# zkemail/zk-email-verify

Measured on NVIDIA H100. Metric: EmailVerifier proofs/sec (witness+prove), higher is better.
Workload: dtype u256 (BN254 Fr/Fq integers, 8x32-bit limbs)

## Files before the change

### zk-email-verify_b200/csrc/engine.cu

```cuda
#include "ff.cuh"
namespace zke { namespace dev { unsigned long long g_kernel_launches = 0; } }
#include "witness.cu"
#include "matvec.cu"
#include "ntt.cu"
#include "msm.cuh"
#include "fixed_base.cuh"
namespace zke { namespace dev {
ZKE_DEFINE_CONSTANT_UPLOAD(upload_constants_engine)
cudaError_t upload_constants_msm_g1(const FieldConsts*, const FieldConsts*);
cudaError_t upload_constants_msm_g2(const FieldConsts*, const FieldConsts*);
cudaError_t upload_constants_fixed_base(const FieldConsts*, const FieldConsts*);
cudaError_t upload_constants_verify(const FieldConsts*, const FieldConsts*);
} }

#include "../../include/zkemail_b200.h"
#include "cuda_host.hpp"
#include "engine.hpp"
#include "witness_program.hpp"
#include "binfile.hpp"
#include "ec_host.hpp"
#include "setup_host.hpp"
#include <algorithm>
#include <cstdio>
#include <cstring>
// ... 766 lines not shown
static void sync_lanes(zke_ctx* x) {
    cudaStreamSynchronize(x->stream);
    for (int i = 0; i < x->lanes_alloc; ++i) { cudaStreamSynchronize(x->lanes[i].st); cudaStreamSynchronize(x->lanes[i].heavy); }
}

static void enqueue_prove(zke_ctx* x, zke_ctx::Slot& S, size_t batch, const uint8_t* rs) {
    const zke_zkey* zk = x->zkey;
    if (!zk) throw std::runtime_error("context was opened without a proving key");
    if (batch == 0 || batch > S.loaded) throw std::runtime_error("no witness loaded for this batch (call zke_witness first)");
    if (rs) {
        for (size_t e = 0; e < 2 * batch; ++e) {
            U256 v;
            memcpy(v.v, rs + 32 * e, 32);
            if (u256_cmp(v, fr_params().p) >= 0) throw std::runtime_error("r / s not reduced mod the group order");
        }
        S.rs.assign(rs, rs + 64 * batch);
    } else {
        S.rs.clear();
    }
    CUDA_OK(cudaSetDevice(x->device));
    const uint32_t N = 1u << zk->log_n, m = x->n_vars, l = x->n_public;
    const bool prof = x->profile;
    const int n_lanes = prof ? 1 : x->n_lanes;
    if (const char* e = getenv("ZKE_SPLIT_STREAMS")) x->split_streams = atoi(e) != 0;
    if (l) CUDA_OK(cudaMemcpy2DAsync(S.publics_host, (size_t)l * 32, S.w_all.p + 32, x->stride * 32, (size_t)l * 32, batch, cudaMemcpyDeviceToHost, x->stream));
    CUDA_OK(cudaEventRecord(S.witness_done, x->stream));
    for (int i = 0; i < n_lanes; ++i) CUDA_OK(cudaStreamWaitEvent(x->lanes[i].st, S.witness_done, 0));
    for (size_t e = 0; e < batch; ++e) {
        zke_ctx::Lane& L = x->lanes[e % n_lanes];
        cudaStream_t st = L.st;
        const uint8_t* w = S.w_all.p + 32 * x->stride * e;
        uint8_t* res = S.results.p + (size_t)ZKE_RESULT_STRIDE * e;
        uint32_t* flag = (uint32_t*)(res + ZKE_RES_FLAG_OFF);
        size_t t0 = 0, t1 = 0;
        CUDA_OK(cudaMemsetAsync(flag, 0xff, 4, st));
        if (prof) t0 = x->mark(st);
        cudaStream_t hv = (prof || !x->split_streams) ? st : L.heavy;
        dev::launch_build_ab(x->r1cs, w, L.va.p, L.vb.p, L.vc.p, N, flag, st);
        if (prof) { t1 = x->mark(st); x->spans.push_back({ZKE_STAGE_MATVEC, t0, t1}); t0 = t1; }
        if (hv != st) { CUDA_OK(cudaEventRecord(L.ev[0], st)); CUDA_OK(cudaStreamWaitEvent(hv, L.ev[0], 0)); }
        dev::launch_intt_dif(L.va.p, x->ntt, x->coset_scale.p, hv);
        dev::launch_intt_dif(L.vb.p, x->ntt, x->coset_scale.p, hv);
        dev::launch_intt_dif(L.vc.p, x->ntt, x->coset_scale.p, hv);
        dev::launch_ntt_dit(L.va.p, x->ntt, hv);
        dev::launch_ntt_dit(L.vb.p, x->ntt, hv);
        dev::launch_ntt_dit(L.vc.p, x->ntt, hv);
        dev::launch_quotient(L.va.p, L.vb.p, L.vc.p, L.vd.p, N, hv);
        CHECK_LAUNCH();
        if (hv != st) CUDA_OK(cudaEventRecord(L.ev[1], hv));
        if (prof) { t1 = x->mark(st); x->spans.push_back({ZKE_STAGE_NTT, t0, t1}); t0 = t1; }
        uint8_t* ws_w = L.msm_ws.p;
        dev::MsmPlan<dev::Fq>::run(zk->A.p, w, m, x->cfg_w, ws_w, res + 0 * ZKE_RES_G1_BLOCK, st);
        if (prof) { t1 = x->mark(st); x->spans.push_back({ZKE_STAGE_MSM_A, t0, t1}); t0 = t1; }
        dev::MsmPlan<dev::Fq>::run(zk->B1.p, w, m, x->cfg_w, ws_w, res + 1 * ZKE_RES_G1_BLOCK, st);
        if (prof) { t1 = x->mark(st); x->spans.push_back({ZKE_STAGE_MSM_B1, t0, t1}); t0 = t1; }
        dev::MsmPlan<dev::Fq>::run(zk->C.p, w, m, x->cfg_w, ws_w, res + 2 * ZKE_RES_G1_BLOCK, st);
        if (prof) { t1 = x->mark(st); x->spans.push_back({ZKE_STAGE_MSM_C, t0, t1}); t0 = t1; }
        dev::MsmPlan<dev::Fq2>::run(zk->B2.p, w, m, x->cfg_w, ws_w, res + 4 * ZKE_RES_G1_BLOCK, st);
        CHECK_LAUNCH();
        if (prof) { t1 = x->mark(st); x->spans.push_back({ZKE_STAGE_MSM_B2, t0, t1}); t0 = t1; }
        if (hv != st) CUDA_OK(cudaStreamWaitEvent(st, L.ev[1], 0));
        {
            dev::MsmPlan<dev::Fq>::Heavy heavy{hv, L.ev[2], L.ev[3]};
            if (prof) {
                size_t i0, i1;
                cudaEvent_t evs[2];
                evs[0] = x->ev(&i0); evs[1] = x->ev(&i1);
                dev::MsmPlan<dev::Fq>::run(zk->H.p, L.vd.p, N, x->cfg_h, L.msm_ws.p, res + 3 * ZKE_RES_G1_BLOCK, st, evs, &heavy);
                x->spans.push_back({ZKE_STAGE_MSM_H_BUCKETS, i0, i1});
                t1 = x->mark(st); x->spans.push_back({ZKE_STAGE_MSM_H, t0, t1}); t0 = t1;
            } else {
                dev::MsmPlan<dev::Fq>::run(zk->H.p, L.vd.p, N, x->cfg_h, L.msm_ws.p, res + 3 * ZKE_RES_G1_BLOCK, st, nullptr, &heavy);
            }
        }
        CHECK_LAUNCH();
        CUDA_OK(cudaMemcpyAsync(S.results_host + (size_t)ZKE_RESULT_STRIDE * e, res, ZKE_RESULT_STRIDE, cudaMemcpyDeviceToHost, st));
        CUDA_OK(cudaEventRecord(S.done[e], st));
    }
    S.batch = (uint32_t)batch;
}

static int finish_prove(zke_ctx* x, zke_ctx::Slot& S, uint8_t* proofs_out, uint8_t* publics_out, int32_t* status, std::string& msg) {
    const zke_zkey* zk = x->zkey;
    const size_t batch = S.batch;
    const uint32_t l = x->n_public;
    const G1JacH alpha1 = G1JacH::from_affine(zk->alpha1), beta1 = G1JacH::from_affine(zk->beta1), delta1 = G1JacH::from_affine(zk->delta1);
    const G2JacH beta2 = G2JacH::from_affine(zk->beta2), delta2 = G2JacH::from_affine(zk->delta2);
    std::vector<int32_t> st_local(batch, -1);
    std::string first_error;
    std::mutex err_mutex;
    auto one = [&](size_t e) {
        CUDA_OK(cudaEventSynchronize(S.done[e]));
        const uint8_t* res = S.results_host + (size_t)ZKE_RESULT_STRIDE * e;
        uint32_t flag;
        memcpy(&flag, res + ZKE_RES_FLAG_OFF, 4);
        const int32_t s = flag == 0xffffffffu ? -1 : (int32_t)flag;
        st_local[e] = s;
        uint8_t* out = proofs_out + 256 * e;
        if (s >= 0) { memset(out, 0, 256); return; }
        U256 r, sc;
        if (!S.rs.empty()) { memcpy(r.v, S.rs.data() + 64 * e, 32); memcpy(sc.v, S.rs.data() + 64 * e + 32, 32); }
        else { random_scalar(r); random_scalar(sc); }
        G1AffineH ma = finish_msm<Fq>(res + 0 * ZKE_RES_G1_BLOCK, x->cfg_w);
        G1AffineH mb1 = finish_msm<Fq>(res + 1 * ZKE_RES_G1_BLOCK, x->cfg_w);
        G1AffineH mc = finish_msm<Fq>(res + 2 * ZKE_RES_G1_BLOCK, x->cfg_w);
        G1AffineH mh = finish_msm<Fq>(res + 3 * ZKE_RES_G1_BLOCK, x->cfg_h);
        G2AffineH mb2 = finish_msm<Fq2>(res + 4 * ZKE_RES_G1_BLOCK, x->cfg_w);
        G1JacH pa = alpha1.add(G1JacH::from_affine(ma)).add(delta1.mul(r));
        G2JacH pb2 = beta2.add(G2JacH::from_affine(mb2)).add(delta2.mul(sc));
        G1JacH pb1 = beta1.add(G1JacH::from_affine(mb1)).add(delta1.mul(sc));
        U256 rs_prod = (Fr::from_u256(r) * Fr::from_u256(sc)).to_u256();
        G1JacH pc = G1JacH::from_affine(mc).add(G1JacH::from_affine(mh)).add(pa.mul(sc)).add(pb1.mul(r)).add(delta1.mul(rs_prod).neg());
        G1AffineH A = pa.to_affine(), C = pc.to_affine();
// ... 110 lines not shown
    map.log_cols = log_cols; map.log_m = log_m; map.col0 = col0;
    const uint32_t n_rows = (uint32_t)world << log_cols;
    dev::launch_build_ab(x->r1cs, S.w_all.p, L.va.p, L.vb.p, L.vc.p, n_rows, flag, st, &map);
    const uint32_t n_cols = 1u << log_cols;
    dev::launch_intt_cross(L.va.p, x->ntt, log_g, col0, n_cols, st);
    dev::launch_intt_cross(L.vb.p, x->ntt, log_g, col0, n_cols, st);
    dev::launch_intt_cross(L.vc.p, x->ntt, log_g, col0, n_cols, st);
    CHECK_LAUNCH();
    CUDA_OK(cudaStreamSynchronize(st));
    x->shard_stage = 1;
}

static void shard_mid(zke_ctx* x) {
    if (x->shard_stage != 1) throw std::runtime_error("zke_shard_mid out of order");
    CUDA_OK(cudaSetDevice(x->device));
    int log_m, log_cols; uint32_t col0;
    shard_geometry(x, log_m, log_cols, col0);
    zke_ctx::Lane& L = x->lanes[0];
    cudaStream_t st = L.st;
    const size_t block_off = ((size_t)x->shard_rank << log_m);
    for (uint8_t* v : {L.va.p, L.vb.p, L.vc.p}) {
        dev::launch_intt_dif_block(v + 32 * block_off, x->ntt, log_m, x->coset_scale.p + (x->ntt.shoup ? 64 : 32) * block_off, st);
        dev::launch_ntt_dit_block(v + 32 * block_off, x->ntt, log_m, st);
    }
    CHECK_LAUNCH();
    CUDA_OK(cudaStreamSynchronize(st));
    x->shard_stage = 2;
}

static void put_g1(uint8_t* dst, const G1AffineH& p) { write_fq(dst, p.x); write_fq(dst + 32, p.y); }

static void shard_end(zke_ctx* x, uint8_t* partial_out, uint8_t* publics_out) {
    if (x->shard_stage != 2) throw std::runtime_error("zke_shard_end out of order");
    const zke_zkey* zk = x->zkey;
    CUDA_OK(cudaSetDevice(x->device));
    int log_m, log_cols; uint32_t col0;
    shard_geometry(x, log_m, log_cols, col0);
    zke_ctx::Slot& S = x->slots[0];
    zke_ctx::Lane& L = x->lanes[0];
    cudaStream_t st = L.st;
    const uint32_t N = 1u << zk->log_n, m = x->n_vars, l = x->n_public;
    const int G = x->shard_world, log_g = x->shard_log_g;
    const uint32_t n_cols = 1u << log_cols;
    dev::launch_ntt_cross(L.va.p, x->ntt, log_g, col0, n_cols, st);
    dev::launch_ntt_cross(L.vb.p, x->ntt, log_g, col0, n_cols, st);
    dev::launch_ntt_cross(L.vc.p, x->ntt, log_g, col0, n_cols, st);
    CUDA_OK(cudaMemsetAsync(L.vd.p, 0, (size_t)N * 32, st));
    dev::launch_quotient_cols(L.va.p, L.vb.p, L.vc.p, L.vd.p, (int)zk->log_n, log_g, col0, (uint32_t)log_cols, st);
    CHECK_LAUNCH();
    const uint32_t lo = (uint32_t)((uint64_t)m * x->shard_rank / G), hi = (uint32_t)((uint64_t)m * (x->shard_rank + 1) / G);
    const uint8_t* w = S.w_all.p;
    uint8_t* res = S.results.p;
    dev::MsmPlan<dev::Fq>::run(zk->A.p + 64ull * lo, w + 32ull * lo, hi - lo, x->cfg_w, L.msm_ws.p, res + 0 * ZKE_RES_G1_BLOCK, st);
    dev::MsmPlan<dev::Fq>::run(zk->B1.p + 64ull * lo, w + 32ull * lo, hi - lo, x->cfg_w, L.msm_ws.p, res + 1 * ZKE_RES_G1_BLOCK, st);
    dev::MsmPlan<dev::Fq>::run(zk->C.p + 64ull * lo, w + 32ull * lo, hi - lo, x->cfg_w, L.msm_ws.p, res + 2 * ZKE_RES_G1_BLOCK, st);
    dev::MsmPlan<dev::Fq2>::run(zk->B2.p + 128ull * lo, w + 32ull * lo, hi - lo, x->cfg_w, L.msm_ws.p, res + 4 * ZKE_RES_G1_BLOCK, st);
    dev::MsmPlan<dev::Fq>::run(zk->H.p, L.vd.p, N, x->cfg_h, L.msm_ws.p, res + 3 * ZKE_RES_G1_BLOCK, st);
    CHECK_LAUNCH();
    CUDA_OK(cudaMemcpyAsync(S.results_host, res, ZKE_RESULT_STRIDE, cudaMemcpyDeviceToHost, st));
    if (l) CUDA_OK(cudaMemcpyAsync(S.publics_host, S.w_all.p + 32, (size_t)l * 32, cudaMemcpyDeviceToHost, st));
    CUDA_OK(cudaStreamSynchronize(st));
    const uint8_t* rh = S.results_host;
    put_g1(partial_out + 0, finish_msm<Fq>(rh + 0 * ZKE_RES_G1_BLOCK, x->cfg_w));
    put_g1(partial_out + 64, finish_msm<Fq>(rh + 1 * ZKE_RES_G1_BLOCK, x->cfg_w));
    put_g1(partial_out + 128, finish_msm<Fq>(rh + 2 * ZKE_RES_G1_BLOCK, x->cfg_w));
    put_g1(partial_out + 192, finish_msm<Fq>(rh + 3 * ZKE_RES_G1_BLOCK, x->cfg_h));
    const G2AffineH b2 = finish_msm<Fq2>(rh + 4 * ZKE_RES_G1_BLOCK, x->cfg_w);
    write_fq(partial_out + 256, b2.x.c0); write_fq(partial_out + 288, b2.x.c1); write_fq(partial_out + 320, b2.y.c0); write_fq(partial_out + 352, b2.y.c1);
    memcpy(partial_out + 384, rh + ZKE_RES_FLAG_OFF, 4);
    if (publics_out && l) memcpy(publics_out, S.publics_host, (size_t)l * 32);
    x->shard_stage = 0;
}

static Fq fq_from_le(const uint8_t* b) {
    U256 v;
    memcpy(v.v, b, 32);
    if (u256_cmp(v, fq_params().p) >= 0) throw std::runtime_error("partial point coordinate not reduced");
    return Fq::from_u256(v);
}

struct ShardKeyPoints { G1AffineH alpha1, beta1, delta1; G2AffineH beta2, delta2; };
static int shard_combine(const ShardKeyPoints* zk, const uint8_t* partials, int world, const uint8_t* rs, uint8_t* out, int32_t* status) {
    G1JacH sa = G1JacH::inf(), sb1 = G1JacH::inf(), sc = G1JacH::inf(), sh = G1JacH::inf();
    G2JacH sb2 = G2JacH::inf();
    uint32_t first_bad = 0xffffffffu;
    for (int r = 0; r < world; ++r) {
        const uint8_t* p = partials + (size_t)ZKE_SHARD_PARTIAL_BYTES * r;
        auto g1 = [&](const uint8_t* q) { return G1AffineH{fq_from_le(q), fq_from_le(q + 32)}; };
        const G1AffineH a = g1(p), b1 = g1(p + 64), c = g1(p + 128), h = g1(p + 192);
        const G2AffineH b2{Fq2{fq_from_le(p + 256), fq_from_le(p + 288)}, Fq2{fq_from_le(p + 320), fq_from_le(p + 352)}};
        if (!g1_on_curve(a) || !g1_on_curve(b1) || !g1_on_curve(c) || !g1_on_curve(h) || !g2_on_curve(b2)) throw std::runtime_error("partial point not on the curve");
        sa = sa.add_affine(a); sb1 = sb1.add_affine(b1); sc = sc.add_affine(c); sh = sh.add_affine(h); sb2 = sb2.add_affine(b2);
        uint32_t f;
        memcpy(&f, p + 384, 4);
        first_bad = std::min(first_bad, f);
    }
    if (status) *status = first_bad == 0xffffffffu ? -1 : (int32_t)first_bad;
    if (first_bad != 0xffffffffu) { memset(out, 0, 256); return 1; }
    U256 r, s;
    if (rs) { memcpy(r.v, rs, 32); memcpy(s.v, rs + 32, 32); }
    else { random_scalar(r); random_scalar(s); }
    if (u256_cmp(r, fr_params().p) >= 0 || u256_cmp(s, fr_params().p) >= 0) throw std::runtime_error("r / s not reduced mod the group order");
    const G1JacH alpha1 = G1JacH::from_affine(zk->alpha1), beta1 = G1JacH::from_affine(zk->beta1), delta1 = G1JacH::from_affine(zk->delta1);
    const G2JacH beta2 = G2JacH::from_affine(zk->beta2), delta2 = G2JacH::from_affine(zk->delta2);
    G1JacH pa = alpha1.add(sa).add(delta1.mul(r));
    G2JacH pb2 = beta2.add(sb2).add(delta2.mul(s));
    G1JacH pb1 = beta1.add(sb1).add(delta1.mul(s));
    U256 rs_prod = (Fr::from_u256(r) * Fr::from_u256(s)).to_u256();
    G1JacH pc = sc.add(sh).add(pa.mul(s)).add(pb1.mul(r)).add(delta1.mul(rs_prod).neg());
// ... 315 lines not shown
```

### zk-email-verify_b200/csrc/msm.cu

```cuda
#include "device_engine.cuh"
#include "msm.cuh"
#include "msm_ba.cuh"
#include "msm_sort.cuh"
#if defined(ZKE_MSM_G1)
#include "msm_tc.cuh"
#endif
#include <algorithm>
#include <cstdlib>
#include <stdexcept>

namespace zke {
namespace dev {

static const int LIST_FANIN = 32;
static const int TREE_FANIN = 8;

__device__ __forceinline__ Fr load_scalar(const uint8_t* scalars, uint32_t i) { return Fr::load(scalars + 32ull * i); }

template <class F>
__global__ void classify_kernel(const uint8_t* __restrict__ points, const uint8_t* __restrict__ scalars, uint32_t n,
                                uint32_t* ones_list, uint32_t* gen_list, uint32_t* counters ) {
    const uint32_t i = blockIdx.x * blockDim.x + threadIdx.x;
    if (i >= n) return;
    Fr s = load_scalar(scalars, i);
    if (s.is_zero()) return;
    Affine<F> p = Affine<F>::load(points + sizeof(Affine<F>) * (size_t)i);
    if (p.is_inf()) return;
    bool one = s.v[0] == 1 && (s.v[1] | s.v[2] | s.v[3] | s.v[4] | s.v[5] | s.v[6] | s.v[7]) == 0;
    if (one) ones_list[atomicAdd(&counters[0], 1u)] = i;
    else gen_list[atomicAdd(&counters[1], 1u)] = i;
}

template <class F>
__global__ void sum_affine_list_kernel(const uint8_t* __restrict__ points, const uint32_t* __restrict__ list,
                                       const uint32_t* __restrict__ count_ptr, uint32_t count_fixed, uint8_t* out) {
    const uint32_t count = count_ptr ? *count_ptr : count_fixed;
    const uint32_t t = blockIdx.x * blockDim.x + threadIdx.x;
    const uint32_t n_out = max(1u, (count + LIST_FANIN - 1) / LIST_FANIN);
    if (t >= n_out) return;
    XYZZ<F> acc = XYZZ<F>::inf();
    for (uint32_t k = t; k < count; k += n_out) {
        uint32_t idx = list ? list[k] : k;
        acc.madd(Affine<F>::load(points + sizeof(Affine<F>) * (size_t)idx), false);
    }
    acc.store(out + sizeof(XYZZ<F>) * (size_t)t);
}

__device__ __forceinline__ uint32_t tree_level_size(uint32_t count, uint32_t level) {
    uint32_t n = max(1u, (count + LIST_FANIN - 1) / LIST_FANIN);
    for (uint32_t d = 0; d < level; ++d) n = max(1u, (n + TREE_FANIN - 1) / TREE_FANIN);
    return n;
}
template <class F>
__global__ void sum_xyzz_kernel(const uint8_t* __restrict__ in, const uint32_t* __restrict__ count_ptr, uint32_t count_fixed,
                                uint32_t level, uint32_t pad_to, uint8_t* out) {
    const uint32_t count = count_ptr ? *count_ptr : count_fixed;
    const uint32_t n_in = tree_level_size(count, level), n_out = tree_level_size(count, level + 1);
    const uint32_t t = blockIdx.x * blockDim.x + threadIdx.x;
    if (t >= n_out) {
        if (t < pad_to) XYZZ<F>::inf().store(out + sizeof(XYZZ<F>) * (size_t)t);
        return;
    }
    XYZZ<F> acc = XYZZ<F>::inf();
    for (uint32_t k = t; k < n_in; k += n_out) acc.add(XYZZ<F>::load(in + sizeof(XYZZ<F>) * (size_t)k));
    acc.store(out + sizeof(XYZZ<F>) * (size_t)t);
}

struct Digits {
    int c, n_windows;
    uint32_t half;
    uint32_t chunk;
    uint32_t group;
    uint32_t window_bucket_stride;
    uint32_t window_point_stride;
};

__device__ __forceinline__ uint32_t window_bits(const Fr& s, int bit, int c) {
    const int w = bit >> 5, b = bit & 31;
    uint64_t two = s.v[w];
    if (w + 1 < 8) two |= (uint64_t)s.v[w + 1] << 32;
// ... 513 lines not shown
    const Affine<F>* in = sorted0;
    Affine<F>* out = ping;
    for (int l = 0; l < L; ++l) {
        const size_t slots = BaPlan<F>::slots_bound(max_entries, n_buckets, l + 1);
        const uint32_t n_threads = (uint32_t)((slots + BA_K - 1) / BA_K);
        const uint32_t blocks = (n_threads + BA_THREADS - 1) / BA_THREADS;
        fill_work_kernel<<<(n_buckets + 255) / 256, 256, 0, st>>>(hist, off[l + 1], n_buckets, 1u << (l + 1), 0, slot_bucket);
        BaLevel lv{hist, off[l], off[l + 1], slot_bucket, n_buckets, (uint32_t)l};
        to_heavy();
        if (ev && l == 0) cudaEventRecord(ev[0], hv);
        ba_forward_kernel<F><<<blocks, BA_THREADS, 0, hv>>>(lv, in, prefix, tot, n_threads);
        to_light();
        batch_inverse<F>(tot, n_threads, binv_scratch, st);
        to_heavy();
        ba_backward_kernel<F><<<blocks, BA_THREADS, 0, hv>>>(lv, in, prefix, tot, out, n_threads);
        if (ev && l == L - 1) cudaEventRecord(ev[1], hv);
        to_light();
        ZKE_COUNT_LAUNCH(3);
        in = out;
        out = (out == ping) ? pong : ping;
    }
    XYZZ<F>* bucket_sum = (XYZZ<F>*)sorted0;
    bucket_finish_kernel<F><<<(n_buckets + 127) / 128, 128, 0, st>>>(in, hist, off[L], n_buckets, (uint32_t)L, bucket_sum);
    group_sum_kernel<F, 1><<<(groups + 127) / 128, 128, 0, st>>>((const uint8_t*)bucket_sum, hist, off[L], D.half, groups, 1u << L, 0, D.group, group_out);
    ZKE_COUNT_LAUNCH(2);
}
template <>
void run_ba<Fq2>(const MsmConfig&, const uint32_t*, const uint32_t*, uint32_t, size_t, uint32_t*, uint8_t*, const Digits&,
                 uint32_t, uint8_t*, cudaStream_t, cudaEvent_t*, const MsmPlan<Fq2>::Heavy*) {}

#if defined(ZKE_MSM_G1)
MsmConfig msm_config_witness() {
    MsmConfig c; c.c = 8; c.chunk = 32; c.group = 8; c.classify = true; c.extra_passes = 2;
    if (const char* e = getenv("ZKE_W_C")) c.c = std::max(4, std::min(16, atoi(e)));
    if (const char* e = getenv("ZKE_W_CHUNK")) c.chunk = (uint32_t)std::max(8, atoi(e));
    if (const char* e = getenv("ZKE_W_GROUP")) c.group = (uint32_t)std::max(2, atoi(e));
    return c;
}
MsmConfig msm_config_full(uint32_t n, bool precomputed) {
    MsmConfig c;
    c.c = n >= (1u << 18) ? 16 : (n >= (1u << 12) ? 12 : 8);
    c.chunk = 256; c.group = n >= (1u << 20) ? 64 : 16; c.classify = false; c.extra_passes = 0;
    c.precomputed = precomputed;
    c.ba_levels = 0;
    if (const char* e = getenv("ZKE_H_BA")) c.ba_levels = precomputed ? std::max(0, std::min(6, atoi(e))) : 0;
    if (const char* e = getenv("ZKE_H_GROUP")) c.group = (uint32_t)std::max(2, atoi(e));
    if (precomputed) {
        c.c = n >= (1u << 20) ? 20 : (n >= (1u << 16) ? 17 : (n >= (1u << 10) ? 12 : 8));
    }
    return c;
}
#endif

template <class F>
size_t MsmPlan<F>::workspace_bytes(uint32_t n, const MsmConfig& cfg) {
    const int W = (255 + cfg.c - 1) / cfg.c;
    const size_t half = (size_t)1 << (cfg.c - 1);
    const size_t bucket_sets = cfg.precomputed ? 1 : W;
    const size_t n_buckets = half * bucket_sets;
    const size_t max_entries = (size_t)n * W;
    const size_t max_chunks = n_buckets + max_entries / cfg.chunk + 1;
    const size_t groups = ((half + cfg.group - 1) / cfg.group) * bucket_sets;
    size_t b = 0;
    auto al = [&](size_t x) { b += (x + 255) & ~(size_t)255; };
    al(4 * 2);
    al(4 * (size_t)n);
    al(4 * (size_t)n);
    al(4 * (n_buckets + 1));
    al(4 * (n_buckets + 1));
    al(4 * (n_buckets + 1));
    al(4 * (n_buckets / SCAN_TILE + 2));
    al(4 * max_entries);
    al(4 * max_chunks);
    al(sizeof(XYZZ<F>) * max_chunks);
    al(sizeof(XYZZ<F>) * (max_chunks / PASS_FANIN + n_buckets + 1));
    al(4 * (n_buckets + 1));
    al(sizeof(XYZZ<F>) * groups);
    al(sizeof(XYZZ<F>) * ((size_t)n / LIST_FANIN + 2) * 2);
    if (cfg.ba_levels > 0 && sizeof(F) == 32) al(BaPlan<F>::bytes(max_entries, n_buckets, cfg.ba_levels));
    const size_t order_cells = ((max_chunks + ORDER_BLOCK - 1) / ORDER_BLOCK) * cfg.chunk;
    al(4 * max_chunks);
    al(4 * (order_cells + 1));
    al(4 * (order_cells + 1));
    al(4 * (order_cells / SCAN_TILE + 2));
    if (n_buckets >= SORT_TWO_LEVEL_MIN_BUCKETS) DigitSort((uint32_t)n, W, (uint32_t)n_buckets, max_entries).place([&](size_t x) { al(x); return (uint8_t*)nullptr; });
    else al(4 * (n_buckets + 1));
    return b;
}

template <class F>
void MsmPlan<F>::run(const uint8_t* points, const uint8_t* scalars, uint32_t n, const MsmConfig& cfg, uint8_t* ws,
                     uint8_t* result, cudaStream_t st, cudaEvent_t* ev, const Heavy* heavy) {
    Digits D;
    D.c = cfg.c;
    D.n_windows = (255 + cfg.c - 1) / cfg.c;
    D.half = 1u << (cfg.c - 1);
    D.chunk = cfg.chunk;
    D.group = cfg.group;
    D.window_bucket_stride = cfg.precomputed ? 0 : D.half;
    D.window_point_stride = cfg.precomputed ? n : 0;
    if (D.n_windows > MSM_MAX_WINDOWS) return;
    const uint32_t bucket_sets = cfg.precomputed ? 1 : (uint32_t)D.n_windows;
    const uint32_t n_buckets = D.half * bucket_sets;
    const size_t max_entries = (size_t)n * D.n_windows;
    const size_t max_chunks = n_buckets + max_entries / cfg.chunk + 1;
    const uint32_t groups_per_window = (D.half + D.group - 1) / D.group;
    const uint32_t groups = groups_per_window * bucket_sets;
    uint8_t* p = ws;
    auto take = [&](size_t x) { uint8_t* r = p; p += (x + 255) & ~(size_t)255; return r; };
    uint32_t* counters = (uint32_t*)take(8);
    uint32_t* ones_list = (uint32_t*)take(4 * (size_t)n);
    uint32_t* gen_list = (uint32_t*)take(4 * (size_t)n);
    uint32_t* hist = (uint32_t*)take(4 * ((size_t)n_buckets + 1));
    uint32_t* offsets = (uint32_t*)take(4 * ((size_t)n_buckets + 1));
    uint32_t* chunk_off = (uint32_t*)take(4 * ((size_t)n_buckets + 1));
    uint32_t* tiles = (uint32_t*)take(4 * ((size_t)n_buckets / SCAN_TILE + 2));
    uint32_t* entries = (uint32_t*)take(4 * max_entries);
    uint32_t* work_bucket = (uint32_t*)take(4 * max_chunks);
    uint8_t* partial = take(sizeof(XYZZ<F>) * max_chunks);
    uint8_t* partial2 = take(sizeof(XYZZ<F>) * (max_chunks / PASS_FANIN + n_buckets + 1));
    uint32_t* off2 = (uint32_t*)take(4 * ((size_t)n_buckets + 1));
    uint8_t* group_out = take(sizeof(XYZZ<F>) * groups);
    const size_t list_slots = (size_t)n / LIST_FANIN + 2;
    uint8_t* red_a = take(sizeof(XYZZ<F>) * list_slots);
    uint8_t* red_b = take(sizeof(XYZZ<F>) * list_slots);
    const bool use_ba = cfg.ba_levels > 0 && sizeof(F) == 32;
    uint8_t* ba_ws = use_ba ? take(BaPlan<F>::bytes(max_entries, n_buckets, cfg.ba_levels)) : nullptr;
    const size_t order_cells = ((max_chunks + ORDER_BLOCK - 1) / ORDER_BLOCK) * cfg.chunk;
    uint32_t* order = (uint32_t*)take(4 * max_chunks);
    uint32_t* order_mat = (uint32_t*)take(4 * (order_cells + 1));
    uint32_t* order_off = (uint32_t*)take(4 * (order_cells + 1));
    uint32_t* order_tiles = (uint32_t*)take(4 * (order_cells / SCAN_TILE + 2));
    const bool two_level = n_buckets >= SORT_TWO_LEVEL_MIN_BUCKETS;
    DigitSort sort(n, D.n_windows, n_buckets, max_entries);
    if (sort.fine_bits > SORT_MAX_FINE_BITS) throw std::runtime_error("MSM bucket sort: more than 2^19 buckets");
    uint32_t* cursor = nullptr;
    if (two_level) sort.place(take);
    else cursor = (uint32_t*)take(4 * ((size_t)n_buckets + 1));

    uint8_t* res_ones = result;
    uint8_t* res_windows = result + sizeof(XYZZ<F>) * MSM_ONES_SLOTS;
    cudaMemsetAsync(result, 0, sizeof(XYZZ<F>) * MSM_RESULT_SLOTS, st);

    const uint32_t* gen_count = nullptr;
    const uint32_t* gen_idx = nullptr;
    if (cfg.classify) {
        cudaMemsetAsync(counters, 0, 8, st);
        classify_kernel<F><<<(n + 255) / 256, 256, 0, st>>>(points, scalars, n, ones_list, gen_list, counters);
        uint32_t upper = (n + LIST_FANIN - 1) / LIST_FANIN;
        sum_affine_list_kernel<F><<<(upper + 127) / 128, 128, 0, st>>>(points, ones_list, counters, 0, red_a);
        ZKE_COUNT_LAUNCH(2);
        uint8_t *src = red_a, *dst = red_b;
        uint32_t level = 0;
        for (;;) {
            const uint32_t next = (upper + TREE_FANIN - 1) / TREE_FANIN;
            const bool last = next <= MSM_ONES_SLOTS;
            uint8_t* out = last ? res_ones : dst;
            const uint32_t threads = last ? (uint32_t)MSM_ONES_SLOTS : next;
            sum_xyzz_kernel<F><<<(threads + 63) / 64, 64, 0, st>>>(src, counters, 0, level, last ? MSM_ONES_SLOTS : 0, out);
            ZKE_COUNT_LAUNCH(1);
            if (last) break;
            uint8_t* t = src; src = dst; dst = t;
            upper = next;
            ++level;
        }
        gen_count = counters + 1;
        gen_idx = gen_list;
    }
    const int sms = sm_count();
    if (two_level) {
        sort.run(scalars, gen_idx, gen_count, n, D, hist, offsets, entries, st);
    } else {
        cudaMemsetAsync(hist, 0, 4 * ((size_t)n_buckets + 1), st);
        cudaMemsetAsync(cursor, 0, 4 * ((size_t)n_buckets + 1), st);
        digit_hist_kernel<<<sms * 8, 256, 0, st>>>(scalars, gen_idx, gen_count, n, D, hist);
        exclusive_scan(hist, n_buckets, 0, 0, offsets, tiles, st);
        digit_scatter_kernel<<<sms * 8, 256, 0, st>>>(scalars, gen_idx, gen_count, n, D, offsets, cursor, entries);
        ZKE_COUNT_LAUNCH(2);
    }
    if (use_ba) {
        gather_points_kernel<F><<<sms * 8, 256, 0, st>>>(entries, offsets, n_buckets, points, (Affine<F>*)ba_ws);
        ZKE_COUNT_LAUNCH(1);
        run_ba<F>(cfg, hist, offsets, n_buckets, max_entries, tiles, ba_ws, D, groups, group_out, st, ev, heavy);
    } else {
        exclusive_scan(hist, n_buckets, D.chunk, 0, chunk_off, tiles, st);
        fill_work_kernel<<<(n_buckets + 255) / 256, 256, 0, st>>>(hist, chunk_off, n_buckets, D.chunk, 0, work_bucket);
        {
            const uint32_t nblk = (uint32_t)((max_chunks + ORDER_BLOCK - 1) / ORDER_BLOCK);
            chunk_key_hist_kernel<<<nblk, ORDER_BLOCK, 4 * D.chunk, st>>>(hist, chunk_off, work_bucket, n_buckets, D.chunk, order_mat);
            exclusive_scan(order_mat, nblk * D.chunk, 0, 0, order_off, order_tiles, st);
            chunk_order_kernel<<<nblk, ORDER_BLOCK, 0, st>>>(hist, chunk_off, work_bucket, n_buckets, D.chunk, order_off, order);
            ZKE_COUNT_LAUNCH(2);
        }
        cudaStream_t st_light = st;
        if (heavy && heavy->st != st) {
            cudaEventRecord(heavy->before, st);
            cudaStreamWaitEvent(heavy->st, heavy->before, 0);
            st = heavy->st;
        }
        if (ev) cudaEventRecord(ev[0], st);
        {
            int minb = sizeof(F) == 32 ? 5 : 4, waves = 4;
            if (const char* e = getenv("ZKE_CHUNK_MINB")) minb = atoi(e);
            if (const char* e = getenv("ZKE_CHUNK_WAVES")) waves = std::max(1, atoi(e));
            bool done = false;
#if defined(ZKE_MSM_G1)
            const char* h_tc_env = getenv("ZKE_H_TC");
            const int h_tc = h_tc_env ? atoi(h_tc_env) : 0;
            if (h_tc > 0 && cfg.precomputed) {
                if (const TcTable* tab = tc_table_fq()) {
                    const uint8_t* pts = reinterpret_cast<const uint8_t*>(points);
                    if (h_tc >= 5) chunk_sum_tc_kernel<5><<<sms * 5 * waves, 128, 0, st>>>(pts, entries, offsets, hist, chunk_off, work_bucket, order, n_buckets, D.chunk, partial, tab);
                    else if (h_tc == 4) chunk_sum_tc_kernel<4><<<sms * 4 * waves, 128, 0, st>>>(pts, entries, offsets, hist, chunk_off, work_bucket, order, n_buckets, D.chunk, partial, tab);
                    else chunk_sum_tc_kernel<3><<<sms * 3 * waves, 128, 0, st>>>(pts, entries, offsets, hist, chunk_off, work_bucket, order, n_buckets, D.chunk, partial, tab);
                    done = true;
                }
            }
#endif
            size_t pad = 0;
            if (const char* e = getenv("ZKE_CHUNK_PAD_SMEM")) pad = (size_t)std::max(0, std::min(48 * 1024, atoi(e)));
            if (done) {}
            else if (minb >= 6) chunk_sum_kernel<F, 6><<<sms * 6 * waves, 128, pad, st>>>(points, entries, offsets, hist, chunk_off, work_bucket, order, n_buckets, D.chunk, partial);
            else if (minb == 5) chunk_sum_kernel<F, 5><<<sms * 5 * waves, 128, pad, st>>>(points, entries, offsets, hist, chunk_off, work_bucket, order, n_buckets, D.chunk, partial);
            else chunk_sum_kernel<F, 4><<<sms * 4 * waves, 128, pad, st>>>(points, entries, offsets, hist, chunk_off, work_bucket, order, n_buckets, D.chunk, partial);
        }
        if (ev) cudaEventRecord(ev[1], st);
        if (st != st_light) {
            cudaEventRecord(heavy->after, st);
            cudaStreamWaitEvent(st_light, heavy->after, 0);
            st = st_light;
        }
        uint8_t *items = partial, *items_next = partial2;
        uint32_t *off_cur = chunk_off, *off_next = off2;
        uint32_t levels = 0;
        for (uint32_t pass = 0; pass < cfg.extra_passes; ++pass) {
            exclusive_scan(hist, n_buckets, D.chunk, levels + 1, off_next, tiles, st);
            fill_work_kernel<<<(n_buckets + 255) / 256, 256, 0, st>>>(hist, off_next, n_buckets, D.chunk, levels + 1, work_bucket);
            partial_pass_kernel<F><<<sms * 4, 128, 0, st>>>(items, hist, off_cur, off_next, work_bucket, n_buckets, D.chunk, levels, items_next);
            ZKE_COUNT_LAUNCH(2);
            uint8_t* t = items; items = items_next; items_next = t;
            uint32_t* o = off_cur; off_cur = off_next; off_next = o;
            ++levels;
        }
        group_sum_kernel<F, 0><<<(groups + 127) / 128, 128, 0, st>>>(items, hist, off_cur, D.half, groups, D.chunk, levels, D.group, group_out);
    }
    window_reduce_kernel<F><<<bucket_sets, 512, 0, st>>>(group_out, groups_per_window);
    gather_windows_kernel<F><<<1, 64, 0, st>>>(group_out, groups_per_window, bucket_sets, res_windows);
    ZKE_COUNT_LAUNCH(5);
}

#if defined(ZKE_MSM_G1)
template struct MsmPlan<Fq>;
#elif defined(ZKE_MSM_G2)
template struct MsmPlan<Fq2>;
#else
#error "compile msm.cu through msm_g1.cu / msm_g2.cu"
#endif

}
}
```

### zk-email-verify_b200/csrc/msm.cuh

```cuda
#pragma once
#include "ec.cuh"

namespace zke {
namespace dev {

struct MsmConfig {
    int c = 16;
    uint32_t chunk = 256;
    uint32_t group = 16;
    bool classify = false;
    uint32_t extra_passes = 0;
    bool precomputed = false;
    int ba_levels = 0;
};
MsmConfig msm_config_witness();
MsmConfig msm_config_full(uint32_t n, bool precomputed);
inline int msm_windows(const MsmConfig& c) { return (255 + c.c - 1) / c.c; }

static const int MSM_ONES_SLOTS = 32;
static const int MSM_MAX_WINDOWS = 32;
static const int MSM_RESULT_SLOTS = MSM_ONES_SLOTS + MSM_MAX_WINDOWS;

template <class F>
struct MsmPlan {
    static size_t workspace_bytes(uint32_t n, const MsmConfig& cfg);
    struct Heavy { cudaStream_t st; cudaEvent_t before, after; };
    static void run(const uint8_t* points, const uint8_t* scalars, uint32_t n, const MsmConfig& cfg, uint8_t* workspace,
                    uint8_t* result, cudaStream_t st, cudaEvent_t* ev = nullptr, const Heavy* heavy = nullptr);
};

}
}
```

Baseline: 47.77.

## Reuse B1 scalar classification and bucket sort for the B2 MSM

The B1 (G1) and B2 (G2) MSMs use the same witness scalars. B2 now runs right after B1 in the same workspace and skips classify, digit sort, chunk ordering and per-pass offset computation, taking the index layout B1 left behind. Classify now drops a point only when both its G1 and G2 twins are at infinity, so the shared lists stay correct for both curves. The workspace layout is pulled into a shared struct so both field instantiations place the index arrays at the same offsets. The pass-offset scans are hoisted before the bucket kernels. This relies on workspace layout matching between the G1 and G2 instantiations and on B1 not taking the BA path.

```diff
diff --git a/zk-email-verify_b200/csrc/engine.cu b/zk-email-verify_b200/csrc/engine.cu
--- a/zk-email-verify_b200/csrc/engine.cu
+++ b/zk-email-verify_b200/csrc/engine.cu
@@ -842,13 +842,13 @@
         uint8_t* ws_w = L.msm_ws.p;
         dev::MsmPlan<dev::Fq>::run(zk->A.p, w, m, x->cfg_w, ws_w, res + 0 * ZKE_RES_G1_BLOCK, st);
         if (prof) { t1 = x->mark(st); x->spans.push_back({ZKE_STAGE_MSM_A, t0, t1}); t0 = t1; }
-        dev::MsmPlan<dev::Fq>::run(zk->B1.p, w, m, x->cfg_w, ws_w, res + 1 * ZKE_RES_G1_BLOCK, st);
+        dev::MsmPlan<dev::Fq>::run(zk->B1.p, w, m, x->cfg_w, ws_w, res + 1 * ZKE_RES_G1_BLOCK, st, nullptr, nullptr, false, zk->B2.p);
         if (prof) { t1 = x->mark(st); x->spans.push_back({ZKE_STAGE_MSM_B1, t0, t1}); t0 = t1; }
+        dev::MsmPlan<dev::Fq2>::run(zk->B2.p, w, m, x->cfg_w, ws_w, res + 4 * ZKE_RES_G1_BLOCK, st, nullptr, nullptr, true);
+        if (prof) { t1 = x->mark(st); x->spans.push_back({ZKE_STAGE_MSM_B2, t0, t1}); t0 = t1; }
         dev::MsmPlan<dev::Fq>::run(zk->C.p, w, m, x->cfg_w, ws_w, res + 2 * ZKE_RES_G1_BLOCK, st);
+        CHECK_LAUNCH();
         if (prof) { t1 = x->mark(st); x->spans.push_back({ZKE_STAGE_MSM_C, t0, t1}); t0 = t1; }
-        dev::MsmPlan<dev::Fq2>::run(zk->B2.p, w, m, x->cfg_w, ws_w, res + 4 * ZKE_RES_G1_BLOCK, st);
-        CHECK_LAUNCH();
-        if (prof) { t1 = x->mark(st); x->spans.push_back({ZKE_STAGE_MSM_B2, t0, t1}); t0 = t1; }
         if (hv != st) CUDA_OK(cudaStreamWaitEvent(st, L.ev[1], 0));
         {
             dev::MsmPlan<dev::Fq>::Heavy heavy{hv, L.ev[2], L.ev[3]};
@@ -1065,9 +1065,10 @@
     const uint8_t* w = S.w_all.p;
     uint8_t* res = S.results.p;
     dev::MsmPlan<dev::Fq>::run(zk->A.p + 64ull * lo, w + 32ull * lo, hi - lo, x->cfg_w, L.msm_ws.p, res + 0 * ZKE_RES_G1_BLOCK, st);
-    dev::MsmPlan<dev::Fq>::run(zk->B1.p + 64ull * lo, w + 32ull * lo, hi - lo, x->cfg_w, L.msm_ws.p, res + 1 * ZKE_RES_G1_BLOCK, st);
+    dev::MsmPlan<dev::Fq>::run(zk->B1.p + 64ull * lo, w + 32ull * lo, hi - lo, x->cfg_w, L.msm_ws.p, res + 1 * ZKE_RES_G1_BLOCK, st, nullptr, nullptr,
+                               false, zk->B2.p + 128ull * lo);
+    dev::MsmPlan<dev::Fq2>::run(zk->B2.p + 128ull * lo, w + 32ull * lo, hi - lo, x->cfg_w, L.msm_ws.p, res + 4 * ZKE_RES_G1_BLOCK, st, nullptr, nullptr, true);
     dev::MsmPlan<dev::Fq>::run(zk->C.p + 64ull * lo, w + 32ull * lo, hi - lo, x->cfg_w, L.msm_ws.p, res + 2 * ZKE_RES_G1_BLOCK, st);
-    dev::MsmPlan<dev::Fq2>::run(zk->B2.p + 128ull * lo, w + 32ull * lo, hi - lo, x->cfg_w, L.msm_ws.p, res + 4 * ZKE_RES_G1_BLOCK, st);
     dev::MsmPlan<dev::Fq>::run(zk->H.p, L.vd.p, N, x->cfg_h, L.msm_ws.p, res + 3 * ZKE_RES_G1_BLOCK, st);
     CHECK_LAUNCH();
     CUDA_OK(cudaMemcpyAsync(S.results_host, res, ZKE_RESULT_STRIDE, cudaMemcpyDeviceToHost, st));
diff --git a/zk-email-verify_b200/csrc/msm.cu b/zk-email-verify_b200/csrc/msm.cu
--- a/zk-email-verify_b200/csrc/msm.cu
+++ b/zk-email-verify_b200/csrc/msm.cu
@@ -18,14 +18,14 @@
 __device__ __forceinline__ Fr load_scalar(const uint8_t* scalars, uint32_t i) { return Fr::load(scalars + 32ull * i); }
 
 template <class F>
-__global__ void classify_kernel(const uint8_t* __restrict__ points, const uint8_t* __restrict__ scalars, uint32_t n,
-                                uint32_t* ones_list, uint32_t* gen_list, uint32_t* counters ) {
+__global__ void classify_kernel(const uint8_t* __restrict__ points, const uint8_t* __restrict__ twin_g2, const uint8_t* __restrict__ scalars,
+                                uint32_t n, uint32_t* ones_list, uint32_t* gen_list, uint32_t* counters ) {
     const uint32_t i = blockIdx.x * blockDim.x + threadIdx.x;
     if (i >= n) return;
     Fr s = load_scalar(scalars, i);
     if (s.is_zero()) return;
     Affine<F> p = Affine<F>::load(points + sizeof(Affine<F>) * (size_t)i);
-    if (p.is_inf()) return;
+    if (p.is_inf() && (!twin_g2 || Affine<Fq2>::load(twin_g2 + sizeof(Affine<Fq2>) * (size_t)i).is_inf())) return;
     bool one = s.v[0] == 1 && (s.v[1] | s.v[2] | s.v[3] | s.v[4] | s.v[5] | s.v[6] | s.v[7]) == 0;
     if (one) ones_list[atomicAdd(&counters[0], 1u)] = i;
     else gen_list[atomicAdd(&counters[1], 1u)] = i;
@@ -645,105 +645,136 @@
 }
 #endif
 
+struct MsmWorkspace {
+    Digits D;
+    uint32_t n, n_buckets, bucket_sets, groups_per_window, groups;
+    size_t max_entries, max_chunks, order_cells, list_slots;
+    bool two_level;
+    uint32_t *counters, *ones_list, *gen_list, *hist, *offsets, *tiles, *entries, *order, *order_mat, *order_off, *order_tiles, *cursor;
+    uint32_t* off[MSM_MAX_PASSES + 1];
+    uint32_t* work[MSM_MAX_PASSES + 1];
+    uint8_t *partial, *partial2, *group_out, *red_a, *red_b, *ba_ws;
+    DigitSort sort;
+    MsmWorkspace(uint32_t n_, const MsmConfig& cfg) : n(n_), sort(n_, (255 + cfg.c - 1) / cfg.c,
+            (1u << (cfg.c - 1)) * (cfg.precomputed ? 1u : (uint32_t)((255 + cfg.c - 1) / cfg.c)), (size_t)n_ * ((255 + cfg.c - 1) / cfg.c)) {
+        D.c = cfg.c;
+        D.n_windows = (255 + cfg.c - 1) / cfg.c;
+        D.half = 1u << (cfg.c - 1);
+        D.chunk = cfg.chunk;
+        D.group = cfg.group;
+        D.window_bucket_stride = cfg.precomputed ? 0 : D.half;
+        D.window_point_stride = cfg.precomputed ? n : 0;
+        bucket_sets = cfg.precomputed ? 1 : (uint32_t)D.n_windows;
+        n_buckets = D.half * bucket_sets;
+        max_entries = (size_t)n * D.n_windows;
+        max_chunks = n_buckets + max_entries / cfg.chunk + 1;
+        groups_per_window = (D.half + D.group - 1) / D.group;
+        groups = groups_per_window * bucket_sets;
+        order_cells = ((max_chunks + ORDER_BLOCK - 1) / ORDER_BLOCK) * cfg.chunk;
+        list_slots = (size_t)n / LIST_FANIN + 2;
+        two_level = n_buckets >= SORT_TWO_LEVEL_MIN_BUCKETS;
+    }
+    template <class F, class Take> void place(const MsmConfig& cfg, Take take) {
+        const size_t nb = (size_t)n_buckets + 1;
+        counters = (uint32_t*)take(4 * 2);
+        ones_list = (uint32_t*)take(4 * (size_t)n);
+        gen_list = (uint32_t*)take(4 * (size_t)n);
+        hist = (uint32_t*)take(4 * nb);
+        offsets = (uint32_t*)take(4 * nb);
+        tiles = (uint32_t*)take(4 * ((size_t)n_buckets / SCAN_TILE + 2));
+        entries = (uint32_t*)take(4 * max_entries);
+        size_t items = max_chunks;
+        for (uint32_t l = 0; l <= cfg.extra_passes; ++l) {
+            off[l] = (uint32_t*)take(4 * nb);
+            work[l] = (uint32_t*)take(4 * items);
+            items = items / PASS_FANIN + n_buckets + 1;
+        }
+        order = (uint32_t*)take(4 * max_chunks);
+        order_mat = (uint32_t*)take(4 * (order_cells + 1));
+        order_off = (uint32_t*)take(4 * (order_cells + 1));
+        order_tiles = (uint32_t*)take(4 * (order_cells / SCAN_TILE + 2));
+        cursor = nullptr;
+        if (two_level) sort.place(take);
+        else cursor = (uint32_t*)take(4 * nb);
+        partial = take(sizeof(XYZZ<F>) * max_chunks);
+        partial2 = take(sizeof(XYZZ<F>) * (max_chunks / PASS_FANIN + n_buckets + 1));
+        group_out = take(sizeof(XYZZ<F>) * groups);
+        red_a = take(sizeof(XYZZ<F>) * list_slots);
+        red_b = take(sizeof(XYZZ<F>) * list_slots);
+        const bool use_ba = cfg.ba_levels > 0 && sizeof(F) == 32;
+        ba_ws = use_ba ? take(BaPlan<F>::bytes(max_entries, n_buckets, cfg.ba_levels)) : nullptr;
+    }
+};
+
 template <class F>
 size_t MsmPlan<F>::workspace_bytes(uint32_t n, const MsmConfig& cfg) {
-    const int W = (255 + cfg.c - 1) / cfg.c;
-    const size_t half = (size_t)1 << (cfg.c - 1);
-    const size_t bucket_sets = cfg.precomputed ? 1 : W;
-    const size_t n_buckets = half * bucket_sets;
-    const size_t max_entries = (size_t)n * W;
-    const size_t max_chunks = n_buckets + max_entries / cfg.chunk + 1;
-    const size_t groups = ((half + cfg.group - 1) / cfg.group) * bucket_sets;
     size_t b = 0;
-    auto al = [&](size_t x) { b += (x + 255) & ~(size_t)255; };
-    al(4 * 2);
-    al(4 * (size_t)n);
-    al(4 * (size_t)n);
-    al(4 * (n_buckets + 1));
-    al(4 * (n_buckets + 1));
-    al(4 * (n_buckets + 1));
-    al(4 * (n_buckets / SCAN_TILE + 2));
-    al(4 * max_entries);
-    al(4 * max_chunks);
-    al(sizeof(XYZZ<F>) * max_chunks);
-    al(sizeof(XYZZ<F>) * (max_chunks / PASS_FANIN + n_buckets + 1));
-    al(4 * (n_buckets + 1));
-    al(sizeof(XYZZ<F>) * groups);
-    al(sizeof(XYZZ<F>) * ((size_t)n / LIST_FANIN + 2) * 2);
-    if (cfg.ba_levels > 0 && sizeof(F) == 32) al(BaPlan<F>::bytes(max_entries, n_buckets, cfg.ba_levels));
-    const size_t order_cells = ((max_chunks + ORDER_BLOCK - 1) / ORDER_BLOCK) * cfg.chunk;
-    al(4 * max_chunks);
-    al(4 * (order_cells + 1));
-    al(4 * (order_cells + 1));
-    al(4 * (order_cells / SCAN_TILE + 2));
-    if (n_buckets >= SORT_TWO_LEVEL_MIN_BUCKETS) DigitSort((uint32_t)n, W, (uint32_t)n_buckets, max_entries).place([&](size_t x) { al(x); return (uint8_t*)nullptr; });
-    else al(4 * (n_buckets + 1));
+    MsmWorkspace(n, cfg).place<F>(cfg, [&](size_t x) { b += (x + 255) & ~(size_t)255; return (uint8_t*)nullptr; });
     return b;
 }
 
 template <class F>
 void MsmPlan<F>::run(const uint8_t* points, const uint8_t* scalars, uint32_t n, const MsmConfig& cfg, uint8_t* ws,
-                     uint8_t* result, cudaStream_t st, cudaEvent_t* ev, const Heavy* heavy) {
-    Digits D;
-    D.c = cfg.c;
-    D.n_windows = (255 + cfg.c - 1) / cfg.c;
-    D.half = 1u << (cfg.c - 1);
-    D.chunk = cfg.chunk;
-    D.group = cfg.group;
-    D.window_bucket_stride = cfg.precomputed ? 0 : D.half;
-    D.window_point_stride = cfg.precomputed ? n : 0;
+                     uint8_t* result, cudaStream_t st, cudaEvent_t* ev, const Heavy* heavy, bool reuse, const uint8_t* twin_g2) {
+    MsmWorkspace W(n, cfg);
+    const Digits& D = W.D;
     if (D.n_windows > MSM_MAX_WINDOWS) return;
-    const uint32_t bucket_sets = cfg.precomputed ? 1 : (uint32_t)D.n_windows;
-    const uint32_t n_buckets = D.half * bucket_sets;
-    const size_t max_entries = (size_t)n * D.n_windows;
-    const size_t max_chunks = n_buckets + max_entries / cfg.chunk + 1;
-    const uint32_t groups_per_window = (D.half + D.group - 1) / D.group;
-    const uint32_t groups = groups_per_window * bucket_sets;
+    if (cfg.extra_passes > MSM_MAX_PASSES) throw std::runtime_error("MSM: more than MSM_MAX_PASSES extra passes");
+    if (W.sort.fine_bits > SORT_MAX_FINE_BITS) throw std::runtime_error("MSM bucket sort: more than 2^19 buckets");
     uint8_t* p = ws;
-    auto take = [&](size_t x) { uint8_t* r = p; p += (x + 255) & ~(size_t)255; return r; };
-    uint32_t* counters = (uint32_t*)take(8);
-    uint32_t* ones_list = (uint32_t*)take(4 * (size_t)n);
-    uint32_t* gen_list = (uint32_t*)take(4 * (size_t)n);
-    uint32_t* hist = (uint32_t*)take(4 * ((size_t)n_buckets + 1));
-    uint32_t* offsets = (uint32_t*)take(4 * ((size_t)n_buckets + 1));
-    uint32_t* chunk_off = (uint32_t*)take(4 * ((size_t)n_buckets + 1));
-    uint32_t* tiles = (uint32_t*)take(4 * ((size_t)n_buckets / SCAN_TILE + 2));
-    uint32_t* entries = (uint32_t*)take(4 * max_entries);
-    uint32_t* work_bucket = (uint32_t*)take(4 * max_chunks);
-    uint8_t* partial = take(sizeof(XYZZ<F>) * max_chunks);
-    uint8_t* partial2 = take(sizeof(XYZZ<F>) * (max_chunks / PASS_FANIN + n_buckets + 1));
-    uint32_t* off2 = (uint32_t*)take(4 * ((size_t)n_buckets + 1));
-    uint8_t* group_out = take(sizeof(XYZZ<F>) * groups);
-    const size_t list_slots = (size_t)n / LIST_FANIN + 2;
-    uint8_t* red_a = take(sizeof(XYZZ<F>) * list_slots);
-    uint8_t* red_b = take(sizeof(XYZZ<F>) * list_slots);
-    const bool use_ba = cfg.ba_levels > 0 && sizeof(F) == 32;
-    uint8_t* ba_ws = use_ba ? take(BaPlan<F>::bytes(max_entries, n_buckets, cfg.ba_levels)) : nullptr;
-    const size_t order_cells = ((max_chunks + ORDER_BLOCK - 1) / ORDER_BLOCK) * cfg.chunk;
-    uint32_t* order = (uint32_t*)take(4 * max_chunks);
-    uint32_t* order_mat = (uint32_t*)take(4 * (order_cells + 1));
-    uint32_t* order_off = (uint32_t*)take(4 * (order_cells + 1));
-    uint32_t* order_tiles = (uint32_t*)take(4 * (order_cells / SCAN_TILE + 2));
-    const bool two_level = n_buckets >= SORT_TWO_LEVEL_MIN_BUCKETS;
-    DigitSort sort(n, D.n_windows, n_buckets, max_entries);
-    if (sort.fine_bits > SORT_MAX_FINE_BITS) throw std::runtime_error("MSM bucket sort: more than 2^19 buckets");
-    uint32_t* cursor = nullptr;
-    if (two_level) sort.place(take);
-    else cursor = (uint32_t*)take(4 * ((size_t)n_buckets + 1));
+    W.place<F>(cfg, [&](size_t x) { uint8_t* r = p; p += (x + 255) & ~(size_t)255; return r; });
+    const uint32_t n_buckets = W.n_buckets, groups = W.groups;
+    uint32_t *hist = W.hist, *offsets = W.offsets, *chunk_off = W.off[0], *work_bucket = W.work[0], *tiles = W.tiles;
+    uint32_t *entries = W.entries, *order = W.order, *counters = W.counters;
+    uint8_t *partial = W.partial, *group_out = W.group_out;
+    const bool use_ba = W.ba_ws != nullptr;
+    if (reuse && (use_ba || !cfg.classify)) throw std::runtime_error("MSM: only the classified (witness) MSMs reuse a scalar layout");
 
     uint8_t* res_ones = result;
     uint8_t* res_windows = result + sizeof(XYZZ<F>) * MSM_ONES_SLOTS;
     cudaMemsetAsync(result, 0, sizeof(XYZZ<F>) * MSM_RESULT_SLOTS, st);
 
-    const uint32_t* gen_count = nullptr;
-    const uint32_t* gen_idx = nullptr;
+    const int sms = sm_count();
+    const uint32_t* gen_count = cfg.classify ? counters + 1 : nullptr;
+    const uint32_t* gen_idx = cfg.classify ? W.gen_list : nullptr;
+    if (!reuse) {
+        if (cfg.classify) {
+            cudaMemsetAsync(counters, 0, 8, st);
+            classify_kernel<F><<<(n + 255) / 256, 256, 0, st>>>(points, twin_g2, scalars, n, W.ones_list, W.gen_list, counters);
+            ZKE_COUNT_LAUNCH(1);
+        }
+        if (W.two_level) {
+            W.sort.run(scalars, gen_idx, gen_count, n, D, hist, offsets, entries, st);
+        } else {
+            cudaMemsetAsync(hist, 0, 4 * ((size_t)n_buckets + 1), st);
+            cudaMemsetAsync(W.cursor, 0, 4 * ((size_t)n_buckets + 1), st);
+            digit_hist_kernel<<<sms * 8, 256, 0, st>>>(scalars, gen_idx, gen_count, n, D, hist);
+            exclusive_scan(hist, n_buckets, 0, 0, offsets, tiles, st);
+            digit_scatter_kernel<<<sms * 8, 256, 0, st>>>(scalars, gen_idx, gen_count, n, D, offsets, W.cursor, entries);
+            ZKE_COUNT_LAUNCH(2);
+        }
+        if (!use_ba) {
+            exclusive_scan(hist, n_buckets, D.chunk, 0, chunk_off, tiles, st);
+            fill_work_kernel<<<(n_buckets + 255) / 256, 256, 0, st>>>(hist, chunk_off, n_buckets, D.chunk, 0, work_bucket);
+            {
+                const uint32_t nblk = (uint32_t)((W.max_chunks + ORDER_BLOCK - 1) / ORDER_BLOCK);
+                chunk_key_hist_kernel<<<nblk, ORDER_BLOCK, 4 * D.chunk, st>>>(hist, chunk_off, work_bucket, n_buckets, D.chunk, W.order_mat);
+                exclusive_scan(W.order_mat, nblk * D.chunk, 0, 0, W.order_off, W.order_tiles, st);
+                chunk_order_kernel<<<nblk, ORDER_BLOCK, 0, st>>>(hist, chunk_off, work_bucket, n_buckets, D.chunk, W.order_off, order);
+                ZKE_COUNT_LAUNCH(3);
+            }
+            for (uint32_t l = 1; l <= cfg.extra_passes; ++l) {
+                exclusive_scan(hist, n_buckets, D.chunk, l, W.off[l], tiles, st);
+                fill_work_kernel<<<(n_buckets + 255) / 256, 256, 0, st>>>(hist, W.off[l], n_buckets, D.chunk, l, W.work[l]);
+                ZKE_COUNT_LAUNCH(1);
+            }
+        }
+    }
     if (cfg.classify) {
-        cudaMemsetAsync(counters, 0, 8, st);
-        classify_kernel<F><<<(n + 255) / 256, 256, 0, st>>>(points, scalars, n, ones_list, gen_list, counters);
         uint32_t upper = (n + LIST_FANIN - 1) / LIST_FANIN;
-        sum_affine_list_kernel<F><<<(upper + 127) / 128, 128, 0, st>>>(points, ones_list, counters, 0, red_a);
-        ZKE_COUNT_LAUNCH(2);
-        uint8_t *src = red_a, *dst = red_b;
+        sum_affine_list_kernel<F><<<(upper + 127) / 128, 128, 0, st>>>(points, W.ones_list, counters, 0, W.red_a);
+        ZKE_COUNT_LAUNCH(1);
+        uint8_t *src = W.red_a, *dst = W.red_b;
         uint32_t level = 0;
         for (;;) {
             const uint32_t next = (upper + TREE_FANIN - 1) / TREE_FANIN;
@@ -757,34 +788,12 @@
             upper = next;
             ++level;
         }
-        gen_count = counters + 1;
-        gen_idx = gen_list;
-    }
-    const int sms = sm_count();
-    if (two_level) {
-        sort.run(scalars, gen_idx, gen_count, n, D, hist, offsets, entries, st);
+    }
+    if (use_ba) {
+        gather_points_kernel<F><<<sms * 8, 256, 0, st>>>(entries, offsets, n_buckets, points, (Affine<F>*)W.ba_ws);
+        ZKE_COUNT_LAUNCH(1);
+        run_ba<F>(cfg, hist, offsets, n_buckets, W.max_entries, tiles, W.ba_ws, D, groups, group_out, st, ev, heavy);
     } else {
-        cudaMemsetAsync(hist, 0, 4 * ((size_t)n_buckets + 1), st);
-        cudaMemsetAsync(cursor, 0, 4 * ((size_t)n_buckets + 1), st);
-        digit_hist_kernel<<<sms * 8, 256, 0, st>>>(scalars, gen_idx, gen_count, n, D, hist);
-        exclusive_scan(hist, n_buckets, 0, 0, offsets, tiles, st);
-        digit_scatter_kernel<<<sms * 8, 256, 0, st>>>(scalars, gen_idx, gen_count, n, D, offsets, cursor, entries);
-        ZKE_COUNT_LAUNCH(2);
-    }
-    if (use_ba) {
-        gather_points_kernel<F><<<sms * 8, 256, 0, st>>>(entries, offsets, n_buckets, points, (Affine<F>*)ba_ws);
-        ZKE_COUNT_LAUNCH(1);
-        run_ba<F>(cfg, hist, offsets, n_buckets, max_entries, tiles, ba_ws, D, groups, group_out, st, ev, heavy);
-    } else {
-        exclusive_scan(hist, n_buckets, D.chunk, 0, chunk_off, tiles, st);
-        fill_work_kernel<<<(n_buckets + 255) / 256, 256, 0, st>>>(hist, chunk_off, n_buckets, D.chunk, 0, work_bucket);
-        {
-            const uint32_t nblk = (uint32_t)((max_chunks + ORDER_BLOCK - 1) / ORDER_BLOCK);
-            chunk_key_hist_kernel<<<nblk, ORDER_BLOCK, 4 * D.chunk, st>>>(hist, chunk_off, work_bucket, n_buckets, D.chunk, order_mat);
-            exclusive_scan(order_mat, nblk * D.chunk, 0, 0, order_off, order_tiles, st);
-            chunk_order_kernel<<<nblk, ORDER_BLOCK, 0, st>>>(hist, chunk_off, work_bucket, n_buckets, D.chunk, order_off, order);
-            ZKE_COUNT_LAUNCH(2);
-        }
         cudaStream_t st_light = st;
         if (heavy && heavy->st != st) {
             cudaEventRecord(heavy->before, st);
@@ -823,23 +832,17 @@
             cudaStreamWaitEvent(st_light, heavy->after, 0);
             st = st_light;
         }
-        uint8_t *items = partial, *items_next = partial2;
-        uint32_t *off_cur = chunk_off, *off_next = off2;
-        uint32_t levels = 0;
+        uint8_t *items = partial, *items_next = W.partial2;
         for (uint32_t pass = 0; pass < cfg.extra_passes; ++pass) {
-            exclusive_scan(hist, n_buckets, D.chunk, levels + 1, off_next, tiles, st);
-            fill_work_kernel<<<(n_buckets + 255) / 256, 256, 0, st>>>(hist, off_next, n_buckets, D.chunk, levels + 1, work_bucket);
-            partial_pass_kernel<F><<<sms * 4, 128, 0, st>>>(items, hist, off_cur, off_next, work_bucket, n_buckets, D.chunk, levels, items_next);
-            ZKE_COUNT_LAUNCH(2);
+            partial_pass_kernel<F><<<sms * 4, 128, 0, st>>>(items, hist, W.off[pass], W.off[pass + 1], W.work[pass + 1], n_buckets, D.chunk, pass, items_next);
+            ZKE_COUNT_LAUNCH(1);
             uint8_t* t = items; items = items_next; items_next = t;
-            uint32_t* o = off_cur; off_cur = off_next; off_next = o;
-            ++levels;
-        }
-        group_sum_kernel<F, 0><<<(groups + 127) / 128, 128, 0, st>>>(items, hist, off_cur, D.half, groups, D.chunk, levels, D.group, group_out);
-    }
-    window_reduce_kernel<F><<<bucket_sets, 512, 0, st>>>(group_out, groups_per_window);
-    gather_windows_kernel<F><<<1, 64, 0, st>>>(group_out, groups_per_window, bucket_sets, res_windows);
-    ZKE_COUNT_LAUNCH(5);
+        }
+        group_sum_kernel<F, 0><<<(groups + 127) / 128, 128, 0, st>>>(items, hist, W.off[cfg.extra_passes], D.half, groups, D.chunk, cfg.extra_passes, D.group, group_out);
+    }
+    window_reduce_kernel<F><<<W.bucket_sets, 512, 0, st>>>(group_out, W.groups_per_window);
+    gather_windows_kernel<F><<<1, 64, 0, st>>>(group_out, W.groups_per_window, W.bucket_sets, res_windows);
+    ZKE_COUNT_LAUNCH(4);
 }
 
 #if defined(ZKE_MSM_G1)
diff --git a/zk-email-verify_b200/csrc/msm.cuh b/zk-email-verify_b200/csrc/msm.cuh
--- a/zk-email-verify_b200/csrc/msm.cuh
+++ b/zk-email-verify_b200/csrc/msm.cuh
@@ -20,13 +20,15 @@
 static const int MSM_ONES_SLOTS = 32;
 static const int MSM_MAX_WINDOWS = 32;
 static const int MSM_RESULT_SLOTS = MSM_ONES_SLOTS + MSM_MAX_WINDOWS;
+static const uint32_t MSM_MAX_PASSES = 4;
 
 template <class F>
 struct MsmPlan {
     static size_t workspace_bytes(uint32_t n, const MsmConfig& cfg);
     struct Heavy { cudaStream_t st; cudaEvent_t before, after; };
     static void run(const uint8_t* points, const uint8_t* scalars, uint32_t n, const MsmConfig& cfg, uint8_t* workspace,
-                    uint8_t* result, cudaStream_t st, cudaEvent_t* ev = nullptr, const Heavy* heavy = nullptr);
+                    uint8_t* result, cudaStream_t st, cudaEvent_t* ev = nullptr, const Heavy* heavy = nullptr, bool reuse = false,
+                    const uint8_t* twin_g2 = nullptr);
 };
 
 }
```

Result: no change. 48.17 (median of 6 runs) (+0.8%).
